# rahulgaur104/ideal-ballooning-solver

Hardware: AMD Instinct MI355X
Metric: field-line eigenvalue solves/sec (N_zeta=512) (higher is better)
Workload: dtype f64; 1 GPU; configs[1] D3D-shape: 16 surfaces x 8 alpha x 8 theta0 = 1024 solves/step/GPU, N_zeta=512 (513 points), geometry-fed scan with fused per-surface argmax (one launch); nonconverged=0, ranks_in_collective=1

## Files before the change

### ideal-ballooning-solver_amd/csrc/ibs_api.hip

```cpp
#include <hip/hip_runtime.h>

#include <dlfcn.h>

#include <cmath>
#include <cstdarg>
#include <cstdio>
#include <cstdlib>
#include <cstring>
#include <limits>
#include <string>
#include <vector>

#include "../../include/ibs.h"
#include "ibs_launch.hpp"
#include "ibs_wave.hpp"
#include "ibs_lbfgsb2.hpp"
#include "ibs_refine.hpp"
#include <chrono>
#include <thread>

namespace ibs {
LaunchTable& launch_table() {
  static LaunchTable t{};
  return t;
// ... 14 lines not shown

static thread_local std::string g_err;
static int fail(int code, const char* fmt, ...) {
  char buf[512];
  va_list ap;
  va_start(ap, fmt);
  vsnprintf(buf, sizeof(buf), fmt, ap);
  va_end(ap);
  g_err = buf;
  return code;
}
#define HIPCHK(expr)                                                                        \
  do {                                                                                      \
    hipError_t e_ = (expr);                                                                 \
    if (e_ != hipSuccess) return fail(IBS_ERR_HIP, "%s -> %s", #expr, hipGetErrorString(e_)); \
  } while (0)

struct ibs_options {
  int force_p = 0;
  int scan_chain = 0;
  int geo_lpp = 0;
  int gcf_rows = -1;
  int gcf_direct = -1;
  int pack_mode = 0;
  int f32_lam = 0;
  double sigma0 = std::numeric_limits<double>::quiet_NaN();
  int sturm_form = 0;
  int reclose = 1;
  int refine_tangent = -1;
  double chain_w1 = 0.25, chain_w2 = 1.0;
  long nearest_chunk_systems = 0;
};

struct ibs_ctx {
  ibs_options opt, opt_created;
  int device = 0;
  hipStream_t stream = nullptr;
  void* ws = nullptr;
  size_t ws_bytes = 0;
  void* hs = nullptr;
  size_t hs_bytes = 0;
  void* long_ws = nullptr;
  size_t long_ws_bytes = 0;
  void* fix_buf = nullptr;
  long fix_cap = 0;
  int lds_per_block = 160 * 1024;
// ... 525 lines not shown
  if (c->fix_buf) hipFree(c->fix_buf);
  for (auto& sc : c->surf_counters) if (sc.buf) hipFree(sc.buf);
  if (c->refine_hist) hipHostFree(c->refine_hist);
  if (c->hs) hipHostFree(c->hs);
  delete c;
  return 0;
}

int ibs_set_stream(ibs_ctx* c, void* s) {
  if (!c) return fail(IBS_ERR_ARG, "null context");
  c->stream = reinterpret_cast<hipStream_t>(s);
  return 0;
}

int ibs_set_option(ibs_ctx* c, const char* name, double value) {
  if (!c || !name) return fail(IBS_ERR_ARG, "null context / name");
  const bool reset = !(value == value);
  const std::string n(name);
  if (n == "force_p") c->opt.force_p = reset ? c->opt_created.force_p : (int)value;
  else if (n == "scan_chain") c->opt.scan_chain = reset ? c->opt_created.scan_chain : (int)value;
  else if (n == "geo_lpp") c->opt.geo_lpp = reset ? c->opt_created.geo_lpp : (int)value;
  else if (n == "gcf_rows") c->opt.gcf_rows = reset ? c->opt_created.gcf_rows : (int)value;
  else if (n == "gcf_direct") c->opt.gcf_direct = reset ? c->opt_created.gcf_direct : (int)value;
  else if (n == "pack_mode") c->opt.pack_mode = reset ? c->opt_created.pack_mode : (int)value;
  else if (n == "f32_lam") c->opt.f32_lam = reset ? c->opt_created.f32_lam : (int)value;
  else if (n == "reclose") c->opt.reclose = reset ? c->opt_created.reclose : (int)value;
  else if (n == "sturm_form") c->opt.sturm_form = reset ? c->opt_created.sturm_form : (int)value;
  else if (n == "sigma0") c->opt.sigma0 = reset ? c->opt_created.sigma0 : value;
  else if (n == "forget_rows") { for (auto& e : c->rows_seen) e = ibs_ctx::RowsSeen{}; }
  else if (n == "refine_tangent") c->opt.refine_tangent = reset ? c->opt_created.refine_tangent : (int)value;
  else if (n == "chain_w1") c->opt.chain_w1 = reset ? c->opt_created.chain_w1 : value;
  else if (n == "chain_w2") c->opt.chain_w2 = reset ? c->opt_created.chain_w2 : value;
  else if (n == "nearest_chunk_systems") c->opt.nearest_chunk_systems = reset ? c->opt_created.nearest_chunk_systems : (long)value;
  else if (n == "all" && reset) c->opt = c->opt_created;
  else return fail(IBS_ERR_ARG, "unknown option '%s'", name);
  return 0;
}

int ibs_lbfgsb2_state_bytes(void) { return (int)sizeof(ibs::lbfgsb2::State); }

int ibs_lbfgsb2_init(void* state, const double* x0, const double* lo, const double* hi, double ftol, double gtol,
                     int32_t maxiter, int32_t maxls) {
  if (!state || !x0 || !lo || !hi) return fail(IBS_ERR_ARG, "null pointer");
  if (!(lo[0] <= hi[0]) || !(lo[1] <= hi[1]) || maxiter < 0 || maxls < 1) return fail(IBS_ERR_ARG, "bad bounds / limits");
  ibs::lbfgsb2::init(*static_cast<ibs::lbfgsb2::State*>(state), x0, lo, hi, ftol, gtol, maxiter, maxls);
  return 0;
// ... 582 lines not shown
  if (G == 1 && !lam_guess && !t0_per_line) {
    const long waves = (long)n_lines * n_theta0, simds = 4L * ctx->n_cu;
    int chain = 1;
    if (n_theta0 >= 8 && waves >= 8 * simds) chain = 4;
    else if (n_theta0 >= 4 && waves >= 4 * simds) chain = 2;
    chain = fit_chain(chain, n_theta0, M, cap);
    if (ctx->opt.scan_chain >= 1 && ctx->opt.scan_chain <= n_theta0) chain = ctx->opt.scan_chain;
    auto fc = ibs::launch_table().scan_chain_f64[M];
    if (chain > 1 && fc) {
      const bool need_x = (M < 3) || X || dX;
      const int wpl = (n_theta0 + chain - 1) / chain;
      long w = need_x ? (long)(((size_t)ctx->lds_per_block - 7 * per_arr) / per_arr) : cap;
      if (w > cap) w = cap;
      if (w > wpl) w = wpl;
      if (w >= 1) {
        const int nb = (wpl + (int)w - 1) / (int)w;
        a.wpb = (wpl + nb - 1) / nb;
        a.chain = chain;
        a.chain_w1 = ctx->opt.chain_w1; a.chain_w2 = ctx->opt.chain_w2;
        fn = fc;
      }
    }
  }
  }
  const size_t n_sys = (size_t)n_lines * n_theta0, in_elems = (size_t)n_lines * ld, out_elems = n_sys * N;
  const size_t n_t0_vals = t0_per_line ? (size_t)n_lines : (size_t)n_theta0;
  a.guess_width = guess_width;
  auto decl = [&](Stage& s) {
    a.bmag = s.in(bmag, in_elems); a.gradpar = s.in(gradpar, in_elems); a.cvdrift = s.in(cvdrift, in_elems);
    a.cvdrift0 = s.in(cvdrift0, in_elems); a.gds2 = s.in(gds2, in_elems); a.gds21 = s.in(gds21, in_elems); a.gds22 = s.in(gds22, in_elems);
    a.dPdrho = s.in(dPdrho, n_lines); a.theta0 = s.in(theta0, n_t0_vals); a.lam_guess = s.in(lam_guess, n_sys);
    a.gam = s.out(gam, n_sys, true); a.lam = s.out(lam, n_sys, true); a.X = s.out(X, out_elems); a.dX = s.out(dX, out_elems);
    a.dth0 = s.out(dth0, n_sys); a.info = s.status(info, n_sys);
  };
  return staged(ctx, mem, decl, [&]() -> int {
    const bool fused = !lng && pack && fn == ibs::launch_table().scan_f64[M] && G == 1;
    if (fused) {
      ibs_ctx::SurfCounters* sc = nullptr;
      for (auto& e : ctx->surf_counters) if (e.stream == ctx->stream) { sc = &e; break; }
      if (!sc) { ctx->surf_counters.push_back(ibs_ctx::SurfCounters{ctx->stream, nullptr, 0}); sc = &ctx->surf_counters.back(); }
      if (sc->n < n_surf) {
        if (sc->buf) { HIPCHK(hipStreamSynchronize(ctx->stream)); HIPCHK(hipFree(sc->buf)); sc->buf = nullptr; sc->n = 0; }
        const int cap_n = n_surf > 1024 ? n_surf : 1024;
        HIPCHK(hipMalloc(reinterpret_cast<void**>(&sc->buf), (size_t)cap_n * sizeof(int)));
        HIPCHK(hipMemsetAsync(sc->buf, 0, (size_t)cap_n * sizeof(int), ctx->stream));
        sc->n = cap_n;
      }
// ... 519 lines not shown
```

### ideal-ballooning-solver_amd/csrc/ibs_kernels.hip

```cpp
#include "ibs_wave.hpp"
#include "ibs_launch.hpp"
#include "ibs_refine.hpp"
#include <type_traits>

#ifndef IBS_M
#error "compile with -DIBS_M=<rows per lane>"
#endif
#ifndef IBS_DIRECT_MIN_M
#define IBS_DIRECT_MIN_M 9
#endif
#ifndef IBS_F32LAM_DIRECT_MIN_M
#define IBS_F32LAM_DIRECT_MIN_M 3
#endif

namespace ibs {

template <typename T>
struct SrcGCF {
  static constexpr bool kHasGh = false;
  const T* gs; const T* cs; const T* fs;
  __device__ __forceinline__ T g(int j) const { return gs[lpos(j)]; }
  __device__ __forceinline__ T c(int j) const { return cs[lpos(j)]; }
  __device__ __forceinline__ T f(int j) const { return fs[lpos(j)]; }
  __device__ __forceinline__ void gcf(int j, T& g_, T& c_, T& f_) const { const int q = lpos(j); g_ = gs[q]; c_ = cs[q]; f_ = fs[q]; }
// ... 34 lines not shown
  static constexpr bool kHasGh = false;
  const T* A1; const T* A3; const T* C0; const T* C1; const T* G0; const T* G1; const T* G2;
  T th0, two_th0, th0sq;
  T cs = T(1);
  __device__ __forceinline__ T sc(T v) const { if constexpr (SCALED) return cs * v; else return v; }
  __device__ __forceinline__ T gd(int j) const { const int q = lpos(j); return G0[q] + two_th0 * G1[q] + th0sq * G2[q]; }
  __device__ __forceinline__ T g(int j) const { return A1[lpos(j)] * gd(j); }
  __device__ __forceinline__ T c(int j) const { const int q = lpos(j); return sc(C0[q] + th0 * C1[q]); }
  __device__ __forceinline__ T f(int j) const { return A3[lpos(j)] * gd(j); }
  __device__ __forceinline__ T gdp(int j) const { const int q = lpos(j); return T(2) * G1[q] + two_th0 * G2[q]; }
  __device__ __forceinline__ T g_t(int j) const { return A1[lpos(j)] * gdp(j); }
  __device__ __forceinline__ T c_t(int j) const { return sc(C1[lpos(j)]); }
  __device__ __forceinline__ T f_t(int j) const { return A3[lpos(j)] * gdp(j); }
  __device__ __forceinline__ void gcf(int j, T& g_, T& c_, T& f_) const {
    const int q = lpos(j);
    const T d = G0[q] + two_th0 * G1[q] + th0sq * G2[q];
    g_ = A1[q] * d; c_ = sc(C0[q] + th0 * C1[q]); f_ = A3[q] * d;
  }
  __device__ __forceinline__ void gcf_with_tangent(int j, T& g_, T& c_, T& f_, T& gt, T& ct, T& ft) const {
    const int q = lpos(j);
    const T g1 = G1[q], g2 = G2[q], a1 = A1[q], a3 = A3[q], c1 = C1[q];
    const T d = G0[q] + two_th0 * g1 + th0sq * g2, dp = T(2) * g1 + two_th0 * g2;
    g_ = a1 * d; c_ = sc(C0[q] + th0 * c1); f_ = a3 * d;
    gt = a1 * dp; ct = sc(c1); ft = a3 * dp;
  }
};


struct NoTangent {};
template <typename U> struct TypeId { using type = U; };

template <typename T>
struct AlphaTangent {
  const T* l; const T* r; long ld;
  T mdP_l, mdP_r, th0, two_th0, th0sq, inv_da;
  __device__ __forceinline__ void gcf(const T* p, T mdP, int j, T& g, T& c, T& f) const {
    const T B = p[j], gp = xabs(p[ld + j]);
    const T cv = p[2 * ld + j] + th0 * p[3 * ld + j];
    const T gd = p[4 * ld + j] + two_th0 * p[5 * ld + j] + th0sq * p[6 * ld + j];
    g = gp * gd / B; c = mdP * cv / (gp * B); f = gd / (B * B) / (gp * B);
  }
  __device__ __forceinline__ void at(int j, T& ga, T& ca, T& fa) const {
    T g1, c1, f1, g2, c2, f2;
    gcf(r, mdP_r, j, g1, c1, f1); gcf(l, mdP_l, j, g2, c2, f2);
    ga = (g1 - g2) * inv_da; ca = (c1 - c2) * inv_da; fa = (f1 - f2) * inv_da;
  }
// ... 78 lines not shown
  }
  if (lane == 0) {
    if (lam_out) lam_out[sys] = (TO)lam;
    if (gam_out) __hip_atomic_store(gam_out + sys, (TO)gam, __ATOMIC_RELAXED, __HIP_MEMORY_SCOPE_AGENT);
    if (info_out) info_out[sys] = inf.iters | (inf.status << 16);
  }
}

template <typename T, class Src, bool WT>
__device__ __forceinline__ void simpson_point(const Src& src, int j, T w, T X, T dX, T& y0, T& y1, T& hc, T& hg, T& hf) {
  const T X2 = w * (X * X), dX2 = w * (dX * dX);
  T g_, c_, f_;
  if constexpr (WT) {
    T gt, ct, ft;
    src.gcf_with_tangent(j, g_, c_, f_, gt, ct, ft);
    hc = xfma(ct, X2, hc); hg = xfma(gt, dX2, hg); hf = xfma(ft, X2, hf);
  } else {
    src.gcf(j, g_, c_, f_);
  }
  y0 += c_ * X2 - g_ * dX2;
  y1 = xfma(f_, X2, y1);
}

template <typename T, int M, class Src, bool HF, int PASSES = 1, typename TO = T>
__device__ __forceinline__ void finish_chunk(WaveSolver<T, M>& ws, Src& src, int N, T h, T* Xs, T lam,
                                             const SolveInfo& inf, long sys, typename TypeId<TO>::type* lam_out,
                                             typename TypeId<TO>::type* gam_out, typename TypeId<TO>::type* X_out,
                                             typename TypeId<TO>::type* dX_out, typename TypeId<TO>::type* dth0_out,
                                             int* info_out, const T* gh = nullptr) {
  static_assert(M >= 3, "the halo exchange takes two rows from each neighbour lane");
  const int lane = ws.lane;
  const int n = N - 2;
  const bool hl = ws.has_last;
  T x[M];
  ws.assemble(src, gh, N, h, x);
  T m = T(0);
#pragma unroll
  for (int i = 0; i < M; ++i) m = xmax(m, xabs(x[i]));
  m = uniform(wave_max(m));
  const T rm = T(1) / m;
#pragma unroll
  for (int i = 0; i < M; ++i) x[i] *= rm;
  int a = WaveSolver<T, M>::rows_start(lane, n);
  asm volatile("" : "+v"(a));
  const T lastv = hl ? x[M - 1] : x[M - 2], last2 = hl ? x[M - 2] : x[M - 3];
  const T xp1 = dpp_t<0x130, 0xF>(T(0), x[0]), xp2 = dpp_t<0x130, 0xF>(T(0), x[1]);
  T xe[M + 4];
  xe[0] = dpp_t<0x138, 0xF>(T(0), last2); xe[1] = dpp_t<0x138, 0xF>(T(0), lastv);
#pragma unroll
  for (int i = 0; i < M - 1; ++i) xe[i + 2] = x[i];
  xe[M + 1] = hl ? x[M - 1] : xp1; xe[M + 2] = hl ? xp1 : xp2; xe[M + 3] = xp2;
  IBS_PROBE_AT(13);
  const T ih = T(1) / h;
  const T A_in = (T(2) / T(3)) * ih, B_in = -ih / T(12), A_e1 = T(0.5) * ih, A_e0 = T(2) * ih, B_e0 = T(-0.5) * ih;
  bool do_hf = false;
  if constexpr (HF) do_hf = dth0_out != nullptr;
  T y0 = T(0), y1 = T(0), hc = T(0), hg = T(0), hf = T(0);
  const T w_even = ((a + 1) & 1) ? T(4) : T(2), w_odd = ((a + 1) & 1) ? T(2) : T(4);
  const int i_end = (lane == kWave - 1) ? (hl ? M - 1 : M - 2) : -1;
  const T dX_end = xfma(A_e0, lane == 0 ? x[0] : -lastv, B_e0 * (lane == 0 ? x[1] : -last2));
  auto all_points = [&](auto with_tangent) {
    if (lane == 0 || lane == kWave - 1)
      simpson_point<T, Src, HF && decltype(with_tangent)::value>(src, lane == 0 ? 0 : N - 1, T(1), T(0), dX_end, y0, y1, hc, hg, hf);
#pragma unroll
    for (int i = 0; i < M; ++i) {
      const bool act = (i < M - 1) || hl;
      const bool e1 = (i == 0 && lane == 0) || (i == i_end);
      const T A = e1 ? A_e1 : A_in, B = e1 ? T(0) : B_in;
      const T dX = xfma(A, xe[i + 3] - xe[i + 1], B * (xe[i + 4] - xe[i]));
      const T w = act ? ((i & 1) ? w_odd : w_even) : T(0);
      simpson_point<T, Src, HF && decltype(with_tangent)::value>(src, a + i + 1, w, xe[i + 2], dX, y0, y1, hc, hg, hf);
      if ((i & 3) == 3) __builtin_amdgcn_sched_barrier(0);
    }
  };
  if constexpr (HF) {
    if (do_hf) all_points(std::true_type{});
    else all_points(std::false_type{});
  } else {
#pragma unroll
    for (int pass = 0; pass < PASSES; ++pass) {
      if constexpr (PASSES > 1) src.begin_pass(pass);
      all_points(std::false_type{});
    }
  }
  IBS_PROBE_AT(14);
  y0 = wave_sum(y0); y1 = wave_sum(y1);
  const T gam = y0 / y1;
  if constexpr (HF) {
    if (do_hf) {
      hc = wave_sum(hc); hg = wave_sum(hg); hf = wave_sum(hf);
      const T jac = hc / y1 - hg / y1 - gam * hf / y1;
      if (lane == 0) dth0_out[sys] = (TO)jac;
    }
  }
  if (lane == 0) {
// ... 621 lines not shown
  if (!gam_out && !X_out && !dX_out) {
    if (lane == 0 && valid) {
      if (lam_out) lam_out[sysc] = (TI)lam;
      if (info_out) info_out[sysc] = inf.iters | (inf.status << 16);
    }
    return;
  }
  src.hold(0);
  finish_chunk<T, M, SrcRows<T, M, TI>, false, 3, TI>(ws, src, N, h, row, lam, inf, sysc, valid ? lam_out : nullptr,
                                                      valid ? gam_out : nullptr, valid ? X_out : nullptr, valid ? dX_out : nullptr,
                                                      nullptr, valid ? info_out : nullptr);
  IBS_PROBE_AT(4);
  if (redo) {
    WaveSolver<T, M> w2;
    (void)setup_rows<T, M, TI>(w2, src, N, h);
    w2.sweep(lam); w2.twisted(lam);
    src.hold(0);
    finish_chunk<T, M, SrcRows<T, M, TI>, false, 3, TI>(w2, src, N, h, row, lam, inf, sysc, valid ? lam_out : nullptr,
                                                        valid ? gam_out : nullptr, valid ? X_out : nullptr, valid ? dX_out : nullptr,
                                                        nullptr, valid ? info_out : nullptr);
  }
}

template <typename T, int M>
__global__ void __launch_bounds__(scan_max_threads(M)) k_gamma_scan(int n_lines, int n_theta0, int N, T h,
                                                     const T* __restrict__ bmag, const T* __restrict__ gradpar,
                                                     const T* __restrict__ cvdrift, const T* __restrict__ cvdrift0,
                                                     const T* __restrict__ gds2, const T* __restrict__ gds21,
                                                     const T* __restrict__ gds22, long ld,
                                                     const T* __restrict__ dPdrho, const T* __restrict__ theta0,
                                                     T* gam_out, T* lam_out, T* X_out, T* dX_out, T* dth0_out,
                                                     int* info_out, const T* __restrict__ lam_guess, T guess_width,
                                                     int lines_per_surf, int* surf_counter, T* pack, int pack_mode,
                                                     int t0_stride) {
  extern __shared__ __align__(16) unsigned char smem_raw[];
  T* smem = reinterpret_cast<T*>(smem_raw);
  const int wave = threadIdx.x >> 6, lane = threadIdx.x & 63;
  const int wpb = blockDim.x >> 6;
  IBS_PROBE_AT(0);
  const int nparts = (n_theta0 + wpb - 1) / wpb;
  int line, part;
  {
    const int b = blockIdx.x;
    const int chunk = b / (8 * nparts), r = b - chunk * 8 * nparts;
    const int lines_here = min(8, n_lines - chunk * 8);
    line = chunk * 8 + r % lines_here;
    part = r / lines_here;
    if (part >= nparts) return;
  }
  const int P = lds_pitch(N);
  T* A1 = smem; T* A3 = A1 + P; T* C0 = A3 + P; T* C1 = C0 + P; T* G0 = C1 + P; T* G1 = G0 + P; T* G2 = G1 + P;
  T* Xs = G2 + P + (size_t)wave * P;
  const int it0 = part * wpb + wave;
  const bool valid = it0 < n_theta0;
  const int it0c = valid ? it0 : (n_theta0 - 1);
  const T th0 = theta0[(long)line * t0_stride + it0c];
  const long sys = (long)line * n_theta0 + it0c;
  const T guess = lam_guess ? lam_guess[sys] : T(0);
  {
    const long off = (long)line * ld;
    const T mdP = -dPdrho[line];
    for (int j = threadIdx.x; j < N; j += blockDim.x) {
      const T B = bmag[off + j], gp = xabs(gradpar[off + j]);
      const T inv = T(1) / (gp * B);
      const int q = lpos(j);
      A1[q] = gp / B;
      A3[q] = inv / (B * B);
      C0[q] = mdP * cvdrift[off + j] * inv;
      C1[q] = mdP * cvdrift0[off + j] * inv;
      G0[q] = gds2[off + j]; G1[q] = gds21[off + j]; G2[q] = gds22[off + j];
    }
  }
  __syncthreads();
  IBS_PROBE_AT(1);
  SrcGeo<T> src{A1, A3, C0, C1, G0, G1, G2, th0, T(2) * th0, th0 * th0};
  WaveSolver<T, M> ws;
  SolveInfo inf{0, 0};
#ifdef IBS_PROBE_TWICE
  { int N2 = N; asm volatile("" : "+s"(N2)); WaveSolver<T, M> w0; (void)w0.template setup<SrcGeo<T>, true>(src, N2, h); asm volatile("" :: "v"(w0.kap), "v"(w0.D[0]), "v"(w0.Ph[M - 1]), "v"(w0.trial_rho)); }
  IBS_PROBE_AT(15);
#endif
  const bool bad = ws.template setup<SrcGeo<T>, true>(src, N, h);
  IBS_PROBE_AT(2);
  T lam = T(0);
  if (!bad) {
    T g_ = guess, w_ = guess_width;
    if (!lam_guess) ws.trial_guess(g_, w_);
    lam = ws.solve(inf, true, g_, w_);
  } else { inf.status = 2; ws.sweep(ws.hi); ws.twisted(ws.hi); }
  IBS_PROBE_AT(3);
  if constexpr (M >= 3) {
    finish_chunk<T, M, SrcGeo<T>, true>(ws, src, N, h, Xs, lam, inf, sys, valid ? lam_out : nullptr,
                                        valid ? gam_out : nullptr, valid ? X_out : nullptr, valid ? dX_out : nullptr,
                                        valid ? dth0_out : nullptr, valid ? info_out : nullptr);
  } else {
    finish<T, M, SrcGeo<T>, true>(ws, src, N, h, Xs, lam, inf, sys, valid ? lam_out : nullptr,
                                  valid ? gam_out : nullptr, valid ? X_out : nullptr, valid ? dX_out : nullptr,
                                  valid ? dth0_out : nullptr, valid ? info_out : nullptr);
  }
  IBS_PROBE_AT(4);
  if (pack) {
    int* flag = reinterpret_cast<int*>(smem + (size_t)(7 + wpb) * P);
    double* sv = reinterpret_cast<double*>(flag + 4);
    int* si = flag + 4 + 2 * 8;
    const int surf = line / lines_per_surf;
    const int nblk_surf = lines_per_surf * nparts;
    asm volatile("s_waitcnt vmcnt(0)" ::: "memory");
    __syncthreads();
    if (threadIdx.x == 0) {
      if (pack_mode != 1) {
        __builtin_amdgcn_fence(__ATOMIC_RELEASE, "agent");
        asm volatile("s_waitcnt vmcnt(0)" ::: "memory");
      }
      const int old = __hip_atomic_fetch_add(&surf_counter[surf], 1, __ATOMIC_RELAXED, __HIP_MEMORY_SCOPE_AGENT);
      const int last = (old == nblk_surf - 1) ? 1 : 0;
      if (last) {
        __hip_atomic_store(&surf_counter[surf], 0, __ATOMIC_RELAXED, __HIP_MEMORY_SCOPE_AGENT);
        if (pack_mode != 1) {
// ... 8 lines not shown
      const int n_per = lines_per_surf * n_theta0;
      const T* gsurf = gam_out + (size_t)surf * n_per;
      T best = -T(1.7976931348623157e308);
      int bi = 0x7fffffff;
      for (int i = threadIdx.x; i < n_per; i += blockDim.x) {
        const T v = __hip_atomic_load(gsurf + i, __ATOMIC_RELAXED, __HIP_MEMORY_SCOPE_AGENT);
        if (v > best || (v == best && i < bi)) { best = v; bi = i; }
      }
#pragma unroll
      for (int d = 32; d >= 1; d >>= 1) {
        const T v2 = __shfl_xor(best, d);
        const int i2 = __shfl_xor(bi, d);
        if (v2 > best || (v2 == best && i2 < bi)) { best = v2; bi = i2; }
      }
      if (lane == 0) { sv[wave] = best; si[wave] = bi; }
      __syncthreads();
      if (threadIdx.x == 0) {
        for (int k = 1; k < wpb; ++k)
          if (sv[k] > best || (sv[k] == best && si[k] < bi)) { best = sv[k]; bi = si[k]; }
        pack[2 * surf] = best; pack[2 * surf + 1] = (T)bi;
      }
    }
  }
}


template <typename T, int M>
__global__ void __launch_bounds__(scan_max_threads(M)) k_gamma_scan_chain(
    int n_lines, int n_theta0, int N, T h, const T* __restrict__ bmag, const T* __restrict__ gradpar,
    const T* __restrict__ cvdrift, const T* __restrict__ cvdrift0, const T* __restrict__ gds2,
    const T* __restrict__ gds21, const T* __restrict__ gds22, long ld, const T* __restrict__ dPdrho,
    const T* __restrict__ theta0, T* gam_out, T* lam_out, T* X_out, T* dX_out, T* dth0_out, int* info_out,
    int chain, T w1, T w2) {
  extern __shared__ __align__(16) unsigned char smem_raw[];
  T* smem = reinterpret_cast<T*>(smem_raw);
  const int wave = threadIdx.x >> 6;
  const int wpb = blockDim.x >> 6;
  const int waves_per_line = (n_theta0 + chain - 1) / chain;
  const int nparts = (waves_per_line + wpb - 1) / wpb;
  int line, part;
  {
    const int b = blockIdx.x;
    const int chunk = b / (8 * nparts), r = b - chunk * 8 * nparts;
    const int lines_here = min(8, n_lines - chunk * 8);
    line = chunk * 8 + r % lines_here;
    part = r / lines_here;
// ... 522 lines not shown
}
#ifdef IBS_WITH_F32
static hipError_t launch_gcf_rows_wide(const GcfArgs<float>& a, hipStream_t st) {
  if constexpr (IBS_M >= 3) {
    const int wpb = a.wpb;
    const size_t lds = (size_t)wpb * lds_pitch(a.N) * sizeof(double);
    const long nblk = (a.n_sys + wpb - 1) / wpb;
    auto kern = k_solve_gcf_rows<double, IBS_M, float>;
    hipError_t e = hipFuncSetAttribute(reinterpret_cast<const void*>(kern), hipFuncAttributeMaxDynamicSharedMemorySize, (int)lds);
    if (e != hipSuccess) return e;
    hipLaunchKernelGGL(kern, dim3((unsigned)nblk), dim3(wpb * 64), lds, st, a.n_sys, a.N, (double)a.h, a.g, a.c, a.f, a.ld,
                       a.lam, a.gam, a.X, a.dX, a.info, a.flags);
    note_launch(nblk, wpb * 64, "ibs::k_solve_gcf_rows<double, %d, float>", IBS_M);
    return hipGetLastError();
  } else {
    return hipErrorInvalidValue;
  }
}
#endif
template <typename T>
static hipError_t launch_scan(const ScanArgs<T>& a, hipStream_t st) {
  const int wpb = a.wpb;
  const size_t lds = (size_t)(7 + wpb) * lds_pitch(a.N) * sizeof(T) + (a.pack ? 128 : 0);
  auto kern = k_gamma_scan<T, IBS_M>;
  hipError_t e = hipFuncSetAttribute(reinterpret_cast<const void*>(kern), hipFuncAttributeMaxDynamicSharedMemorySize, (int)lds);
  if (e != hipSuccess) return e;
  dim3 grid((unsigned)(((a.n_theta0 + wpb - 1) / wpb) * a.n_lines));
  hipLaunchKernelGGL(kern, grid, dim3(wpb * 64), lds, st, a.n_lines, a.n_theta0, a.N, a.h, a.bmag, a.gradpar,
                     a.cvdrift, a.cvdrift0, a.gds2, a.gds21, a.gds22, a.ld, a.dPdrho, a.theta0, a.gam, a.lam, a.X,
                     a.dX, a.dth0, a.info, a.lam_guess, a.guess_width, a.lines_per_surf, a.surf_counter, a.pack, a.pack_mode,
                     a.t0_stride);
  note_launch(grid.x, wpb * 64, "ibs::k_gamma_scan<%s, %d>", type_name<T>(), IBS_M);
  return hipGetLastError();
}
template <typename T>
static hipError_t launch_scan_chain(const ScanArgs<T>& a, hipStream_t st) {
  const int wpb = a.wpb, chain = a.chain;
  const bool need_x = (IBS_M < 3) || a.X || a.dX;
  const size_t lds = (size_t)(7 + (need_x ? wpb : 0)) * lds_pitch(a.N) * sizeof(T);
  auto kern = k_gamma_scan_chain<T, IBS_M>;
  hipError_t e = hipFuncSetAttribute(reinterpret_cast<const void*>(kern), hipFuncAttributeMaxDynamicSharedMemorySize, (int)lds);
  if (e != hipSuccess) return e;
  const int waves_per_line = (a.n_theta0 + chain - 1) / chain;
  dim3 grid((unsigned)(((waves_per_line + wpb - 1) / wpb) * a.n_lines));
  hipLaunchKernelGGL(kern, grid, dim3(wpb * 64), lds, st, a.n_lines, a.n_theta0, a.N, a.h, a.bmag, a.gradpar,
                     a.cvdrift, a.cvdrift0, a.gds2, a.gds21, a.gds22, a.ld, a.dPdrho, a.theta0, a.gam, a.lam, a.X,
                     a.dX, a.dth0, a.info, chain, a.chain_w1, a.chain_w2);
  note_launch(grid.x, wpb * 64, "ibs::k_gamma_scan_chain<%s, %d>", type_name<T>(), IBS_M);
  return hipGetLastError();
}
template <typename T>
static hipError_t launch_sturm(const SturmArgs<T>& a, hipStream_t st) {
  const int wpb = a.wpb;
  const size_t lds = (size_t)wpb * a.N * sizeof(T);
// ... 80 lines not shown
```

### ideal-ballooning-solver_amd/csrc/ibs_launch.hpp

```cpp
#pragma once
#include <hip/hip_runtime.h>
#include <cstdarg>
#include <cstdio>

namespace ibs {

constexpr int kMaxM = 32;
constexpr int kMaxLongN = 65537;

template <typename T>
struct GcfArgs {
  long n_sys; int N; T h; const T* g; const T* c; const T* f; long ld;
  T* lam; T* gam; T* X; T* dX; int* info; int wpb;
  const T* gh;
  int flags;
  int* fix_count; long* fix_sys; double* fix_center;
};
template <typename T>
struct ScanArgs {
  int n_lines, n_theta0, N; T h;
  const T *bmag, *gradpar, *cvdrift, *cvdrift0, *gds2, *gds21, *gds22; long ld;
  const T *dPdrho, *theta0;
  T *gam, *lam, *X, *dX, *dth0; int* info; int wpb;
  const T* lam_guess; T guess_width;
  int chain; T chain_w1, chain_w2;
  int lines_per_surf; int* surf_counter; T* pack;
  int pack_mode;
  int t0_stride;
};
template <typename T>
struct SturmArgs {
  long n_sys; int N; T h; const T* g; const T* c; const T* f; long ld; const T* shift; int* count; int wpb;
};

template <typename T>
struct GradArgs {
  int n_pts, N; T h; const T* geo; long ld; const T* theta0; T del_alpha;
  T *val, *jac, *gam, *dalpha, *dth0; int* info; int wpb;
  long arr_stride, line_stride;
};

struct LongGcfArgs {
  long n_sys; int N; double h;
  const void *g, *c, *f, *gh; int f32;
  long ld; void *lam, *gam, *X, *dX; int* info;
  double* work; int n_waves;
};
hipError_t launch_gcf_long(const LongGcfArgs& a, hipStream_t st);
constexpr size_t nearest_ws_doubles(int N) { return 3 * (size_t)N; }
struct NearestArgs {
  long n_sys; int N; double h;
// ... 152 lines not shown
```

### ideal-ballooning-solver_amd/csrc/ibs_wave.hpp

```cpp
#pragma once
#include <hip/hip_runtime.h>
#include <type_traits>

namespace ibs {

constexpr int kWave = 64;

#ifdef IBS_TRACE_ALL
__device__ double ibs_trace_all[404];
#endif
#ifdef IBS_PROBE
__device__ long long ibs_probe_buf[16 * 4096];
#define IBS_PROBE_AT(k) do { if ((threadIdx.x & 63) == 0 && blockIdx.x < 1024) ibs_probe_buf[(blockIdx.x * 4 + (threadIdx.x >> 6)) * 16 + (k)] = wall_clock64(); } while (0)
#else
#define IBS_PROBE_AT(k) do {} while (0)
#endif



__device__ __forceinline__ int fexp(double x) { return __builtin_amdgcn_frexp_exp(x); }
__device__ __forceinline__ int fexp(float x) { return __builtin_amdgcn_frexp_expf(x); }
__device__ __forceinline__ double xldexp(double x, int e) { return __builtin_ldexp(x, e); }
__device__ __forceinline__ float xldexp(float x, int e) { return __builtin_ldexpf(x, e); }
__device__ __forceinline__ double xfma(double a, double b, double c) { return __builtin_fma(a, b, c); }
// ... 319 lines not shown
    if (top == kWave - 1) { lo = hi; hi = hi + T(64) * w; continue; }
    lo = readlane_t(sig, top); hi = readlane_t(sig, top + 1);
    if (!(hi - lo > stop_eps * epsA)) { ok = true; break; }
  }
  lam = T(0.5) * (lo + hi);
  return ok;
}
template <typename T, class Src>
__device__ __forceinline__ bool multisect_division(const Src& src, int N, T h, T lo, T hi, T normA, int lane, T& lam, int& passes) {
  const T ih2 = T(1) / (h * h);
  return multisect<T>([&](T sig) { return count_above_div<T, Src>(src, N, ih2, sig); }, lo, hi, normA, T(2), lane, lam, passes);
}
template <typename T, class Src>
__device__ __forceinline__ bool reclose_division(const Src& src, int N, T h, T center, T normA, int lane, T& lam, int& passes) {
  const T epsA = Eps<T>::v * normA;
  return multisect_division<T, Src>(src, N, h, center - T(2048) * epsA, center + T(2048) * epsA, normA, lane, lam, passes);
}

struct SolveInfo {
  int iters;
  int status;
};

template <typename T, int M>
struct WaveSolver {
  T D[M], Ph[M];
  T kap, ikap;
  bool has_last;
  int lane;
  T zw[M];
  T u0_in, zu_m1;
  T zw_p1;
  int Eu, Ew;
  T sig_vec;
  T lo, hi, normA;
  T trial_rho, trial_del;
  T trial_mrg;
  T shoot_m; int shoot_e;

  static constexpr int kSetupRows = 4;
  __device__ __forceinline__ static int rows_start(int lane, int n) {
    const int rem = n - kWave * (M - 1);
    return lane * (M - 1) + (lane < rem ? lane : rem);
  }

  template <class Src, bool TRIAL = false>
  __device__ __forceinline__ bool setup(const Src& src, int N, T h) {
    lane = threadIdx.x & (kWave - 1);
    const int n = N - 2;
    const int rem = n - kWave * (M - 1);
    has_last = lane < rem;
    const int a = rows_start(lane, n);
    const T ih2 = T(1) / (h * h);
    T sc = T(1);
    T gcur = T(0);
    T e_lo;
    bool bad = false;
    if constexpr (Src::kHasGh) {
      e_lo = src.gh(a) * ih2;
      bad = !(src.g(a) > T(0));
    } else {
      const T g0 = src.g(a);
      gcur = src.g(a + 1);
      e_lo = T(0.5) * (g0 + gcur) * ih2;
      bad = !(g0 > T(0)) || !(gcur > T(0));
    }
    T vhi = -T(1e300), vlo = -T(1e300), vna = T(0), sum_c = T(0), sum_f = T(0);
    const T e_first = e_lo;
    T ts_prev = T(0), ts_cur = T(0), two_cd = T(0), tA = T(0), tB = T(0), tC = T(0);
    if constexpr (TRIAL) {
      const T dl = T(3.14159265358979323846) / T(N - 1);
      T s0, c0, sd, cd;
      trial_sincos(T(a) * dl, s0, c0);
      trial_sincos(dl, sd, cd);
      ts_prev = s0; ts_cur = xfma(s0, cd, c0 * sd); two_cd = T(2) * cd;
    }
// ... 1 lines not shown
    for (int i = 0; i < M; ++i) {
      const bool act = (i < M - 1) || has_last;
      if (act) {
        const int j = a + i + 1;
        T gnext = T(0), e_hi;
        if constexpr (Src::kHasGh) { e_hi = src.gh(j) * ih2; bad = bad || !(src.g(j + 1) > T(0)); }
        else { gnext = src.g(j + 1); e_hi = T(0.5) * (gcur + gnext) * ih2; bad = bad || !(gnext > T(0)); }
        const T cj = src.c(j), fj = src.f(j);
        const T d = cj - (e_lo + e_hi);
        const T s2 = sc * sc;
        D[i] = d * s2; Ph[i] = fj * s2;
        const T rf = fast_rcp(fj);
        if constexpr (TRIAL) {
          const T ts_next = xfma(two_cd, ts_cur, -ts_prev);
          const T Tx = xfma(e_lo, ts_prev, xfma(d, ts_cur, e_hi * ts_next));
          tA = xfma(ts_cur, Tx, tA); tB = xfma(fj * ts_cur, ts_cur, tB); tC = xfma(Tx * rf, Tx, tC);
          ts_prev = ts_cur; ts_cur = ts_next;
        }
        vhi = xmax(vhi, cj * rf);
        vlo = xmax(vlo, d * rf);
        vna = xmax(vna, (xabs(d) + e_lo + e_hi) * rf);
        sum_c += cj; sum_f += fj;
        bad = bad || !(fj > T(0)) || !(e_hi > T(0)) || !finite_of(cj);
        sc = fast_rcp(e_hi * sc);
        gcur = gnext; e_lo = e_hi;
      } else {
        D[i] = T(0); Ph[i] = T(0);
      }
      if constexpr (M > 8) { if ((i % kSetupRows) == kSetupRows - 1) __builtin_amdgcn_sched_barrier(0); }
    }
    IBS_PROBE_AT(8);
    kap = sc; ikap = fast_rcp(sc);
    bad = bad || !(e_first > T(0));
    const T e0 = readlane_t(e_first, 0);
    const T en = readlane_t(e_lo, kWave - 1);
    const T sc_all = wave_sum(sum_c), sf_all = wave_sum(sum_f);
    normA = uniform(wave_max(vna));
    hi = uniform(wave_max(vhi));
    lo = uniform(xmax(wave_max(vlo), (sc_all - e0 - en) / sf_all));
    hi += T(8) * Eps<T>::v * normA;
    lo -= T(8) * Eps<T>::v * normA;
    if constexpr (TRIAL) {
      const T A = wave_sum(tA), B = wave_sum(tB), C = wave_sum(tC);
      const T rho = A / B;
      trial_rho = rho;
      trial_del = approx_sqrt(xmax(xfma(-rho, A, C), T(0)) / B);
    } else {
      trial_rho = T(0); trial_del = T(-1);
    }
    trial_mrg = T(8 + N / 2) * Eps<T>::v * normA;
// ... 80 lines not shown
    sweep_bwd(sig);
    return c;
  }

  T fu, fw;
  int thr;
  int extra_above;
  template <bool CNT = false>
  __device__ __forceinline__ T twisted(T sig) {
    T best = T(0);
    int bi = 0;
    T zu_b = T(1), zum_b = T(0), zw_b = T(1), zwp_b = T(0), t_b = T(0);
    {
      T zc = u0_in, zp = zu_m1;
#pragma unroll
      for (int i = 0; i < M; ++i) {
        const T t = xfma(-sig, Ph[i], D[i]);
        const bool act = (i < M - 1) || has_last;
        const T a = act ? xabs(Ph[i] * (zc * zw[i])) : T(0);
        const bool better = a > best;
        best = better ? a : best; bi = better ? i : bi;
        zu_b = better ? zc : zu_b; zum_b = better ? zp : zum_b; t_b = better ? t : t_b;
        zw_b = better ? zw[i] : zw_b; zwp_b = better ? (i == M - 1 ? zw_p1 : zw[i < M - 1 ? i + 1 : M - 1]) : zwp_b;
        const T zn = xfma(-t, zc, -zp);
        if (act) { zp = zc; zc = zn; }
      }
    }
    const int ex = expo_of(best);
    constexpr int L = ExpLim<T>::v;
    const int exc = ex < -L ? -L : (ex > L ? L : ex);
    T key = (best > T(0) && finite_of(best) && ex > -(1 << 27)) ? T(ex + Eu + Ew) + T(0.5) * (best * pow2_of<T>(-exc)) : -T(1e30);
    int Lk;
    if constexpr (sizeof(T) == 8) {
      key = __hiloint2double(__double2hiint(key), (__double2loint(key) & ~63) | lane);
      Lk = __double2loint(wave_max(key)) & 63;
    } else {
      key = __int_as_float((__float_as_int(key) & ~63) | lane);
      Lk = __float_as_int(wave_max(key)) & 63;
    }
    const int ik = readlane_i(bi, Lk);
    const T zu_k = readlane_t(zu_b, Lk), zw_k = readlane_t(zw_b, Lk), t_k = readlane_t(t_b, Lk);
    const T um1 = readlane_t(zum_b, Lk), wp1 = readlane_t(zwp_b, Lk);
    const T uw = zu_k * zw_k;
    const T num = xfma(um1, zw_k, xfma(t_k, uw, wp1 * zu_k));
    const int Euk = readlane_i(Eu, Lk), Ewk = readlane_i(Ew, Lk);
    int du = Eu - Euk, dw = Ew - Ewk;
    du = du > 1000 ? 1000 : (du < -2000 ? -2000 : du);
    dw = dw > 1000 ? 1000 : (dw < -2000 ? -2000 : dw);
    fu = xldexp(fast_rcp(zu_k), du);
    fw = xldexp(fast_rcp(zw_k), dw);
    thr = (lane < Lk) ? M : ((lane > Lk) ? -1 : ik);
    T acc = T(0);
    using SignWord = typename std::conditional<(M + 2 <= 32), unsigned, unsigned long long>::type;
    SignWord su = sign_word(zu_m1) >> 31, sw = 0;
    constexpr int MH = M / 2;
    unsigned su_b = 0, sw_a = 0, sw_b = 0, su_a = sign_word(zu_m1) >> 31;
    {
      T zc = u0_in, zp = zu_m1;
#pragma unroll
      for (int i = 0; i < M; ++i) {
        const T t = xfma(-sig, Ph[i], D[i]);
        const bool act = (i < M - 1) || has_last;
        const T xu = zc * fu, xw = zw[i] * fw;
        const T x = (i <= thr) ? xu : xw;
        if (act) acc = xfma(Ph[i] * x, x, acc);
        if constexpr (CNT) {
          if constexpr (sizeof(SignWord) == 4) {
            su = (unsigned)__builtin_amdgcn_alignbit(su, sign_word(zc), 31);
            sw = (unsigned)__builtin_amdgcn_alignbit(sw, sign_word(zw[i]), 31);
          } else if (i < MH) {
            su_a = (unsigned)__builtin_amdgcn_alignbit(su_a, sign_word(zc), 31);
            sw_a = (unsigned)__builtin_amdgcn_alignbit(sw_a, sign_word(zw[i]), 31);
          } else {
            su_b = (unsigned)__builtin_amdgcn_alignbit(su_b, sign_word(zc), 31);
            sw_b = (unsigned)__builtin_amdgcn_alignbit(sw_b, sign_word(zw[i]), 31);
          }
        }
        const T zn = xfma(-t, zc, -zp);
        if (act) { zp = zc; zc = zn; }
      }
    }
    if constexpr (CNT) {
      if constexpr (sizeof(SignWord) == 8) {
        su = ((SignWord)su_a << (M - MH)) | (SignWord)su_b;
        sw = ((SignWord)sw_a << (M - MH)) | (SignWord)sw_b;
      }
      const int last = has_last ? M - 1 : M - 2;
      const int iu = thr < last ? thr : last;
      const SignWord one = 1;
      const SignWord mu = iu >= 0 ? (((one << (iu + 1)) - one) << (M - 1 - iu)) : SignWord(0);
      const int iw = thr > 0 ? thr : 0;
      const SignWord mw = iw <= last ? (((one << (last - iw + 1)) - one) << (M - last)) : SignWord(0);
      const SignWord sw2 = (sw << 1) | (SignWord)(sign_word(zw_p1) >> 31);
      const SignWord fl_u = (su ^ (su >> 1)) & mu, fl_w = (sw2 ^ (sw2 << 1)) & mw;
      int c;
      if constexpr (sizeof(SignWord) == 4) c = __builtin_popcount(fl_u) + __builtin_popcount(fl_w);
      else c = __builtin_popcountll(fl_u) + __builtin_popcountll(fl_w);
      extra_above = wave_sum_i(c);
    }
    sig_vec = sig;
    const T tot = wave_sum(acc);
    return sig + num * fast_rcp(uw * tot);
  }

  template <class Src>
  __device__ __forceinline__ void assemble(const Src& src, const T* gh, int N, T h, T (&x)[M]) {
    int a = rows_start(lane, N - 2);
    asm volatile("" : "+v"(a));
    const T ih2 = T(1) / (h * h);
    T sc = T(1);
    T gcur = src.g(a + 1);
    T zc = u0_in, zp = zu_m1;
#pragma unroll
    for (int i = 0; i < M; ++i) {
      const bool act = (i < M - 1) || has_last;
      const T xu = sc * zc * fu, xw = sc * zw[i] * fw;
      x[i] = act ? ((i <= thr) ? xu : xw) : T(0);
      if (act) {
        T e_hi;
        if (gh) e_hi = gh[a + i + 1] * ih2;
        else { const T gnext = src.g(a + i + 2); e_hi = T(0.5) * (gcur + gnext) * ih2; gcur = gnext; }
        sc = fast_rcp(e_hi * sc);
        const T zn = xfma(-xfma(-sig_vec, Ph[i], D[i]), zc, -zp);
        zp = zc; zc = zn;
      }
      if ((i & 3) == 3) __builtin_amdgcn_sched_barrier(0);
    }
  }

#ifdef IBS_TRACE
  T* trace = nullptr;
#endif
#ifdef IBS_TRACE_ALL
#define IBS_TRACE_SWEEP(it_, sig_, C_, lo_, hi_) do { if (sizeof(T) == 8 && blockIdx.x == 0 && threadIdx.x == 0 && (it_) <= 100) { \
    double* q_ = ibs_trace_all + 4 * ((it_) - 1); q_[0] = (double)(sig_); q_[1] = (double)(C_); q_[2] = (double)(lo_); q_[3] = (double)(hi_); ibs_trace_all[400] = (double)(it_); } } while (0)
#else
#define IBS_TRACE_SWEEP(it_, sig_, C_, lo_, hi_) do {} while (0)
#endif
  struct Pt { T x, m; int e; };
  __device__ __forceinline__ static bool U(bool c) { return __builtin_amdgcn_ballot_w64(c) != 0ull; }
  __device__ __forceinline__ static int uniform_i(int v) { return __builtin_amdgcn_readfirstlane(v); }
  __device__ __forceinline__ static int lg2_of(const Pt& p) { const int e = expo_of(p.m); return e < -(1 << 27) ? e : p.e + e; }
  __device__ __forceinline__ static bool interpolate(const Pt& o, bool use_o, const Pt& a, const Pt& b,
                                                     T lo_, T hi_, T& rho) {
    constexpr int L = ExpLim<T>::v;
    int emax = a.e > b.e ? a.e : b.e;
    if (use_o && o.e > emax) emax = o.e;
// ... 236 lines not shown
```

Measured before the change: 40.84 million solves/s.

## Keep per-row geometry and sweep values resident in registers for small scan grids

Adds a 'resident' variant of the gamma scan kernel that caches per-row geometry factors (a1, d, c, f) and the upward sweep vector in registers during setup and the sweep. Later stages (Rayleigh-quotient recompute, assemble, Simpson finish) then reuse these values instead of reloading from LDS and re-running the recurrence. It also passes precomputed 1/h^2 and 1/h as arguments. The resident path is chosen when the grid is small relative to the CU count, and a lean kernel without these registers is kept for larger grids. The cost is higher register pressure and lower occupancy.

```diff
diff --git a/ideal-ballooning-solver_amd/csrc/ibs_api.hip b/ideal-ballooning-solver_amd/csrc/ibs_api.hip
--- a/ideal-ballooning-solver_amd/csrc/ibs_api.hip
+++ b/ideal-ballooning-solver_amd/csrc/ibs_api.hip
@@ -60,6 +60,7 @@
   int geo_lpp = 0;
   int gcf_rows = -1;
   int gcf_direct = -1;
+  int scan_resident = -1;
   int pack_mode = 0;
   int f32_lam = 0;
   double sigma0 = std::numeric_limits<double>::quiet_NaN();
@@ -631,6 +632,7 @@
   else if (n == "geo_lpp") c->opt.geo_lpp = reset ? c->opt_created.geo_lpp : (int)value;
   else if (n == "gcf_rows") c->opt.gcf_rows = reset ? c->opt_created.gcf_rows : (int)value;
   else if (n == "gcf_direct") c->opt.gcf_direct = reset ? c->opt_created.gcf_direct : (int)value;
+  else if (n == "scan_resident") c->opt.scan_resident = reset ? c->opt_created.scan_resident : (int)value;
   else if (n == "pack_mode") c->opt.pack_mode = reset ? c->opt_created.pack_mode : (int)value;
   else if (n == "f32_lam") c->opt.f32_lam = reset ? c->opt_created.f32_lam : (int)value;
   else if (n == "reclose") c->opt.reclose = reset ? c->opt_created.reclose : (int)value;
@@ -1259,7 +1261,12 @@
       }
     }
   }
-  }
+  if (fn == ibs::launch_table().scan_f64[M] && G == 1) {
+    const long grid_waves = (long)((n_theta0 + a.wpb - 1) / a.wpb) * n_lines * a.wpb;
+    a.resident = ctx->opt.scan_resident == 0 ? 0 : (ctx->opt.scan_resident == 1 ? 1 : (grid_waves <= 2L * 4 * ctx->n_cu ? 1 : 0));
+  }
+  }
+  a.ih2 = 1.0 / (h * h); a.ih = 1.0 / h;
   const size_t n_sys = (size_t)n_lines * n_theta0, in_elems = (size_t)n_lines * ld, out_elems = n_sys * N;
   const size_t n_t0_vals = t0_per_line ? (size_t)n_lines : (size_t)n_theta0;
   a.guess_width = guess_width;
diff --git a/ideal-ballooning-solver_amd/csrc/ibs_kernels.hip b/ideal-ballooning-solver_amd/csrc/ibs_kernels.hip
--- a/ideal-ballooning-solver_amd/csrc/ibs_kernels.hip
+++ b/ideal-ballooning-solver_amd/csrc/ibs_kernels.hip
@@ -80,6 +80,13 @@
     const T g1 = G1[q], g2 = G2[q], a1 = A1[q], a3 = A3[q], c1 = C1[q];
     const T d = G0[q] + two_th0 * g1 + th0sq * g2, dp = T(2) * g1 + two_th0 * g2;
     g_ = a1 * d; c_ = sc(C0[q] + th0 * c1); f_ = a3 * d;
+    gt = a1 * dp; ct = sc(c1); ft = a3 * dp;
+  }
+  __device__ __forceinline__ void g_factors(int j, T& a1, T& d_) const { a1 = A1[lpos(j)]; d_ = gd(j); }
+  __device__ __forceinline__ void tangent(int j, T a1, T& gt, T& ct, T& ft) const {
+    const int q = lpos(j);
+    const T g1 = G1[q], g2 = G2[q], a3 = A3[q], c1 = C1[q];
+    const T dp = T(2) * g1 + two_th0 * g2;
     gt = a1 * dp; ct = sc(c1); ft = a3 * dp;
   }
 };
@@ -204,8 +211,23 @@
   y1 = xfma(f_, X2, y1);
 }
 
-template <typename T, int M, class Src, bool HF, int PASSES = 1, typename TO = T>
-__device__ __forceinline__ void finish_chunk(WaveSolver<T, M>& ws, Src& src, int N, T h, T* Xs, T lam,
+template <typename T, class Src, bool WT>
+__device__ __forceinline__ void simpson_point_carried(const Src& src, int j, T a1, T d_, T c_, T f_, T w, T X, T dX, T& y0, T& y1,
+                                                      T& hc, T& hg, T& hf) {
+  const T X2 = w * (X * X), dX2 = w * (dX * dX);
+  asm volatile("" : "+v"(d_));
+  const T g_ = a1 * d_;
+  if constexpr (WT) {
+    T gt, ct, ft;
+    src.tangent(j, a1, gt, ct, ft);
+    hc = xfma(ct, X2, hc); hg = xfma(gt, dX2, hg); hf = xfma(ft, X2, hf);
+  }
+  y0 += c_ * X2 - g_ * dX2;
+  y1 = xfma(f_, X2, y1);
+}
+
+template <typename T, int M, class Src, bool HF, int PASSES = 1, typename TO = T, bool RES = false>
+__device__ __forceinline__ void finish_chunk(WaveSolver<T, M, RES>& ws, Src& src, int N, T h, T* Xs, T lam,
                                              const SolveInfo& inf, long sys, typename TypeId<TO>::type* lam_out,
                                              typename TypeId<TO>::type* gam_out, typename TypeId<TO>::type* X_out,
                                              typename TypeId<TO>::type* dX_out, typename TypeId<TO>::type* dth0_out,
@@ -233,7 +255,8 @@
   for (int i = 0; i < M - 1; ++i) xe[i + 2] = x[i];
   xe[M + 1] = hl ? x[M - 1] : xp1; xe[M + 2] = hl ? xp1 : xp2; xe[M + 3] = xp2;
   IBS_PROBE_AT(13);
-  const T ih = T(1) / h;
+  T ih;
+  if constexpr (RES) ih = ws.rr.ih; else ih = T(1) / h;
   const T A_in = (T(2) / T(3)) * ih, B_in = -ih / T(12), A_e1 = T(0.5) * ih, A_e0 = T(2) * ih, B_e0 = T(-0.5) * ih;
   bool do_hf = false;
   if constexpr (HF) do_hf = dth0_out != nullptr;
@@ -251,8 +274,14 @@
       const T A = e1 ? A_e1 : A_in, B = e1 ? T(0) : B_in;
       const T dX = xfma(A, xe[i + 3] - xe[i + 1], B * (xe[i + 4] - xe[i]));
       const T w = act ? ((i & 1) ? w_odd : w_even) : T(0);
-      simpson_point<T, Src, HF && decltype(with_tangent)::value>(src, a + i + 1, w, xe[i + 2], dX, y0, y1, hc, hg, hf);
-      if ((i & 3) == 3) __builtin_amdgcn_sched_barrier(0);
+      if constexpr (RES) {
+        simpson_point_carried<T, Src, HF && decltype(with_tangent)::value>(src, a + i + 1, ws.rr.a1[i], ws.rr.d[i], ws.rr.c[i],
+                                                                           ws.rr.f[i], w, xe[i + 2], dX, y0, y1, hc, hg, hf);
+        if constexpr (HF && decltype(with_tangent)::value) { if ((i & 3) == 3) __builtin_amdgcn_sched_barrier(0); }
+      } else {
+        simpson_point<T, Src, HF && decltype(with_tangent)::value>(src, a + i + 1, w, xe[i + 2], dX, y0, y1, hc, hg, hf);
+        if ((i & 3) == 3) __builtin_amdgcn_sched_barrier(0);
+      }
     }
   };
   if constexpr (HF) {
@@ -920,8 +949,8 @@
   }
 }
 
-template <typename T, int M>
-__global__ void __launch_bounds__(scan_max_threads(M)) k_gamma_scan(int n_lines, int n_theta0, int N, T h,
+template <typename T, int M, bool RES>
+__device__ __forceinline__ void gamma_scan_body(int n_lines, int n_theta0, int N, T h,
                                                      const T* __restrict__ bmag, const T* __restrict__ gradpar,
                                                      const T* __restrict__ cvdrift, const T* __restrict__ cvdrift0,
                                                      const T* __restrict__ gds2, const T* __restrict__ gds21,
@@ -930,7 +959,7 @@
                                                      T* gam_out, T* lam_out, T* X_out, T* dX_out, T* dth0_out,
                                                      int* info_out, const T* __restrict__ lam_guess, T guess_width,
                                                      int lines_per_surf, int* surf_counter, T* pack, int pack_mode,
-                                                     int t0_stride) {
+                                                     int t0_stride, T ih2, T ih) {
   extern __shared__ __align__(16) unsigned char smem_raw[];
   T* smem = reinterpret_cast<T*>(smem_raw);
   const int wave = threadIdx.x >> 6, lane = threadIdx.x & 63;
@@ -972,7 +1001,8 @@
   __syncthreads();
   IBS_PROBE_AT(1);
   SrcGeo<T> src{A1, A3, C0, C1, G0, G1, G2, th0, T(2) * th0, th0 * th0};
-  WaveSolver<T, M> ws;
+  WaveSolver<T, M, RES> ws;
+  if constexpr (RES) { ws.rr.ih2 = ih2; ws.rr.ih = ih; }
   SolveInfo inf{0, 0};
 #ifdef IBS_PROBE_TWICE
   { int N2 = N; asm volatile("" : "+s"(N2)); WaveSolver<T, M> w0; (void)w0.template setup<SrcGeo<T>, true>(src, N2, h); asm volatile("" :: "v"(w0.kap), "v"(w0.D[0]), "v"(w0.Ph[M - 1]), "v"(w0.trial_rho)); }
@@ -992,6 +1022,7 @@
                                         valid ? gam_out : nullptr, valid ? X_out : nullptr, valid ? dX_out : nullptr,
                                         valid ? dth0_out : nullptr, valid ? info_out : nullptr);
   } else {
+    static_assert(M >= 3 || !RES, "the resident form lives in finish_chunk");
     finish<T, M, SrcGeo<T>, true>(ws, src, N, h, Xs, lam, inf, sys, valid ? lam_out : nullptr,
                                   valid ? gam_out : nullptr, valid ? X_out : nullptr, valid ? dX_out : nullptr,
                                   valid ? dth0_out : nullptr, valid ? info_out : nullptr);
@@ -1046,6 +1077,39 @@
       }
     }
   }
+}
+
+constexpr bool scan_resident_built(int M) { return M >= 3 && M <= 8; }
+
+template <typename T, int M>
+__global__ void __launch_bounds__(scan_max_threads(M)) k_gamma_scan(int n_lines, int n_theta0, int N, T h,
+                                                     const T* __restrict__ bmag, const T* __restrict__ gradpar,
+                                                     const T* __restrict__ cvdrift, const T* __restrict__ cvdrift0,
+                                                     const T* __restrict__ gds2, const T* __restrict__ gds21,
+                                                     const T* __restrict__ gds22, long ld,
+                                                     const T* __restrict__ dPdrho, const T* __restrict__ theta0,
+                                                     T* gam_out, T* lam_out, T* X_out, T* dX_out, T* dth0_out,
+                                                     int* info_out, const T* __restrict__ lam_guess, T guess_width,
+                                                     int lines_per_surf, int* surf_counter, T* pack, int pack_mode,
+                                                     int t0_stride, T ih2, T ih) {
+  gamma_scan_body<T, M, scan_resident_built(M)>(n_lines, n_theta0, N, h, bmag, gradpar, cvdrift, cvdrift0, gds2, gds21, gds22, ld,
+                                                dPdrho, theta0, gam_out, lam_out, X_out, dX_out, dth0_out, info_out, lam_guess,
+                                                guess_width, lines_per_surf, surf_counter, pack, pack_mode, t0_stride, ih2, ih);
+}
+template <typename T, int M>
+__global__ void __launch_bounds__(scan_max_threads(M)) k_gamma_scan_lean(int n_lines, int n_theta0, int N, T h,
+                                                     const T* __restrict__ bmag, const T* __restrict__ gradpar,
+                                                     const T* __restrict__ cvdrift, const T* __restrict__ cvdrift0,
+                                                     const T* __restrict__ gds2, const T* __restrict__ gds21,
+                                                     const T* __restrict__ gds22, long ld,
+                                                     const T* __restrict__ dPdrho, const T* __restrict__ theta0,
+                                                     T* gam_out, T* lam_out, T* X_out, T* dX_out, T* dth0_out,
+                                                     int* info_out, const T* __restrict__ lam_guess, T guess_width,
+                                                     int lines_per_surf, int* surf_counter, T* pack, int pack_mode,
+                                                     int t0_stride) {
+  gamma_scan_body<T, M, false>(n_lines, n_theta0, N, h, bmag, gradpar, cvdrift, cvdrift0, gds2, gds21, gds22, ld, dPdrho, theta0,
+                               gam_out, lam_out, X_out, dX_out, dth0_out, info_out, lam_guess, guess_width, lines_per_surf,
+                               surf_counter, pack, pack_mode, t0_stride, T(0), T(0));
 }
 
 
@@ -1614,14 +1678,27 @@
 static hipError_t launch_scan(const ScanArgs<T>& a, hipStream_t st) {
   const int wpb = a.wpb;
   const size_t lds = (size_t)(7 + wpb) * lds_pitch(a.N) * sizeof(T) + (a.pack ? 128 : 0);
+  dim3 grid((unsigned)(((a.n_theta0 + wpb - 1) / wpb) * a.n_lines));
+  if constexpr (scan_resident_built(IBS_M)) {
+    if (!a.resident) {
+      auto lean = k_gamma_scan_lean<T, IBS_M>;
+      hipError_t e = hipFuncSetAttribute(reinterpret_cast<const void*>(lean), hipFuncAttributeMaxDynamicSharedMemorySize, (int)lds);
+      if (e != hipSuccess) return e;
+      hipLaunchKernelGGL(lean, grid, dim3(wpb * 64), lds, st, a.n_lines, a.n_theta0, a.N, a.h, a.bmag, a.gradpar,
+                         a.cvdrift, a.cvdrift0, a.gds2, a.gds21, a.gds22, a.ld, a.dPdrho, a.theta0, a.gam, a.lam, a.X,
+                         a.dX, a.dth0, a.info, a.lam_guess, a.guess_width, a.lines_per_surf, a.surf_counter, a.pack, a.pack_mode,
+                         a.t0_stride);
+      note_launch(grid.x, wpb * 64, "ibs::k_gamma_scan_lean<%s, %d>", type_name<T>(), IBS_M);
+      return hipGetLastError();
+    }
+  }
   auto kern = k_gamma_scan<T, IBS_M>;
   hipError_t e = hipFuncSetAttribute(reinterpret_cast<const void*>(kern), hipFuncAttributeMaxDynamicSharedMemorySize, (int)lds);
   if (e != hipSuccess) return e;
-  dim3 grid((unsigned)(((a.n_theta0 + wpb - 1) / wpb) * a.n_lines));
   hipLaunchKernelGGL(kern, grid, dim3(wpb * 64), lds, st, a.n_lines, a.n_theta0, a.N, a.h, a.bmag, a.gradpar,
                      a.cvdrift, a.cvdrift0, a.gds2, a.gds21, a.gds22, a.ld, a.dPdrho, a.theta0, a.gam, a.lam, a.X,
                      a.dX, a.dth0, a.info, a.lam_guess, a.guess_width, a.lines_per_surf, a.surf_counter, a.pack, a.pack_mode,
-                     a.t0_stride);
+                     a.t0_stride, a.ih2, a.ih);
   note_launch(grid.x, wpb * 64, "ibs::k_gamma_scan<%s, %d>", type_name<T>(), IBS_M);
   return hipGetLastError();
 }
diff --git a/ideal-ballooning-solver_amd/csrc/ibs_launch.hpp b/ideal-ballooning-solver_amd/csrc/ibs_launch.hpp
--- a/ideal-ballooning-solver_amd/csrc/ibs_launch.hpp
+++ b/ideal-ballooning-solver_amd/csrc/ibs_launch.hpp
@@ -27,6 +27,7 @@
   int lines_per_surf; int* surf_counter; T* pack;
   int pack_mode;
   int t0_stride;
+  int resident; T ih2, ih;
 };
 template <typename T>
 struct SturmArgs {
diff --git a/ideal-ballooning-solver_amd/csrc/ibs_wave.hpp b/ideal-ballooning-solver_amd/csrc/ibs_wave.hpp
--- a/ideal-ballooning-solver_amd/csrc/ibs_wave.hpp
+++ b/ideal-ballooning-solver_amd/csrc/ibs_wave.hpp
@@ -365,8 +365,17 @@
   int status;
 };
 
+template <typename T, int M, bool RES>
+struct ResidentRows {};
 template <typename T, int M>
+struct ResidentRows<T, M, true> {
+  T a1[M], d[M], c[M], f[M], zu[M];
+  T ih2, ih;
+};
+
+template <typename T, int M, bool RES = false>
 struct WaveSolver {
+  ResidentRows<T, M, RES> rr;
   T D[M], Ph[M];
   T kap, ikap;
   bool has_last;
@@ -394,7 +403,8 @@
     const int rem = n - kWave * (M - 1);
     has_last = lane < rem;
     const int a = rows_start(lane, n);
-    const T ih2 = T(1) / (h * h);
+    T ih2;
+    if constexpr (RES) ih2 = rr.ih2; else ih2 = T(1) / (h * h);
     T sc = T(1);
     T gcur = T(0);
     T e_lo;
@@ -442,10 +452,12 @@
         vna = xmax(vna, (xabs(d) + e_lo + e_hi) * rf);
         sum_c += cj; sum_f += fj;
         bad = bad || !(fj > T(0)) || !(e_hi > T(0)) || !finite_of(cj);
+        if constexpr (RES) { src.g_factors(j, rr.a1[i], rr.d[i]); rr.c[i] = cj; rr.f[i] = fj; }
         sc = fast_rcp(e_hi * sc);
         gcur = gnext; e_lo = e_hi;
       } else {
         D[i] = T(0); Ph[i] = T(0);
+        if constexpr (RES) { rr.a1[i] = T(0); rr.d[i] = T(0); rr.c[i] = T(0); rr.f[i] = T(0); }
       }
       if constexpr (M > 8) { if ((i % kSetupRows) == kSetupRows - 1) __builtin_amdgcn_sched_barrier(0); }
     }
@@ -572,6 +584,7 @@
         best = better ? a : best; bi = better ? i : bi;
         zu_b = better ? zc : zu_b; zum_b = better ? zp : zum_b; t_b = better ? t : t_b;
         zw_b = better ? zw[i] : zw_b; zwp_b = better ? (i == M - 1 ? zw_p1 : zw[i < M - 1 ? i + 1 : M - 1]) : zwp_b;
+        if constexpr (RES) rr.zu[i] = zc;
         const T zn = xfma(-t, zc, -zp);
         if (act) { zp = zc; zc = zn; }
       }
@@ -609,8 +622,8 @@
       T zc = u0_in, zp = zu_m1;
 #pragma unroll
       for (int i = 0; i < M; ++i) {
-        const T t = xfma(-sig, Ph[i], D[i]);
         const bool act = (i < M - 1) || has_last;
+        if constexpr (RES) zc = rr.zu[i];
         const T xu = zc * fu, xw = zw[i] * fw;
         const T x = (i <= thr) ? xu : xw;
         if (act) acc = xfma(Ph[i] * x, x, acc);
@@ -626,8 +639,10 @@
             sw_b = (unsigned)__builtin_amdgcn_alignbit(sw_b, sign_word(zw[i]), 31);
           }
         }
-        const T zn = xfma(-t, zc, -zp);
-        if (act) { zp = zc; zc = zn; }
+        if constexpr (!RES) {
+          const T zn = xfma(-xfma(-sig, Ph[i], D[i]), zc, -zp);
+          if (act) { zp = zc; zc = zn; }
+        }
       }
     }
     if constexpr (CNT) {
@@ -657,13 +672,15 @@
   __device__ __forceinline__ void assemble(const Src& src, const T* gh, int N, T h, T (&x)[M]) {
     int a = rows_start(lane, N - 2);
     asm volatile("" : "+v"(a));
-    const T ih2 = T(1) / (h * h);
+    T ih2;
+    if constexpr (RES) ih2 = rr.ih2; else ih2 = T(1) / (h * h);
     T sc = T(1);
     T gcur = src.g(a + 1);
     T zc = u0_in, zp = zu_m1;
 #pragma unroll
     for (int i = 0; i < M; ++i) {
       const bool act = (i < M - 1) || has_last;
+      if constexpr (RES) zc = rr.zu[i];
       const T xu = sc * zc * fu, xw = sc * zw[i] * fw;
       x[i] = act ? ((i <= thr) ? xu : xw) : T(0);
       if (act) {
@@ -671,8 +688,10 @@
         if (gh) e_hi = gh[a + i + 1] * ih2;
         else { const T gnext = src.g(a + i + 2); e_hi = T(0.5) * (gcur + gnext) * ih2; gcur = gnext; }
         sc = fast_rcp(e_hi * sc);
-        const T zn = xfma(-xfma(-sig_vec, Ph[i], D[i]), zc, -zp);
-        zp = zc; zc = zn;
+        if constexpr (!RES) {
+          const T zn = xfma(-xfma(-sig_vec, Ph[i], D[i]), zc, -zp);
+          zp = zc; zc = zn;
+        }
       }
       if ((i & 3) == 3) __builtin_amdgcn_sched_barrier(0);
     }
```

Measured after the change: 41.73 million solves/s (median of 6 runs). 2.2% higher.
